# a-lemus96/fs-nerf

Hardware: AMD Instinct MI355X
Metric: rendered rays/sec (64+128 samples/ray, 8x256 MLP) (higher is better)
Workload: dtype fp16x3

## Files before the change

fs-nerf_amd/csrc/mlp_dev.hpp:

```cpp
#pragma once
#include "common.hpp"
#include "mlp_layout.hpp"
#ifndef FSN_KLOOP_HEADER
#define FSN_KLOOP_HEADER "kloop_gen.hpp"
#endif
#include FSN_KLOOP_HEADER

#include <type_traits>
#include <utility>

namespace fsn {

typedef __attribute__((ext_vector_type(8))) __bf16 bf16x8;
typedef __attribute__((ext_vector_type(8))) _Float16 f16x8;
typedef __attribute__((ext_vector_type(8))) short s16x8;
typedef __attribute__((ext_vector_type(4))) float f32x4;

constexpr int kNSlot = 4;
constexpr int kLead = 2;
constexpr int kLook = 2;
static_assert(kNSlot >= kLook + 2, "ring safety");
constexpr int kLoaders = 4;
constexpr int kLoaderXor = 4;
constexpr int kOpenVmcnt = (kLook - 1) * (kPhaseBytes / 1024 / kLoaders);
// ... 233 lines not shown
  }
}

constexpr uint32_t kSmallBits = 0x0400u;

struct RangeState {
  uint32_t fmax;
  uint32_t fall;
  uint32_t small;
};

constexpr uint32_t kSmallBitsU = 0x2c00u;

template <bool SMALL, uint32_t BITS = kSmallBits>
__device__ __forceinline__ void range_layer_end(RangeState& r) {
  asm("v_pk_max_u16 %0, %0, %1" : "+v"(r.fall) : "v"(r.fmax));
  if constexpr (SMALL) {
    const uint32_t lo = r.fmax & 0xffffu, hi = r.fmax >> 16;
    const uint32_t m = lo > hi ? lo : hi;
    const int any_big = __builtin_amdgcn_readfirstlane((int)__any(m >= BITS));
    const int any_nz = __builtin_amdgcn_readfirstlane((int)__any(m != 0u));
    if (!any_big && any_nz) r.small = 1u;
  }
  r.fmax = 0u;
}

__device__ __forceinline__ void range_report(uint32_t* status, const RangeState& r, uint32_t range_bit = 1u) {
  const uint32_t f = r.fall;
  const bool bad = (f & 0xffffu) >= 0x7c00u || (f >> 16) >= 0x7c00u;
  uint32_t bits = __builtin_amdgcn_readfirstlane((int)__any(bad)) ? range_bit : 0u;
  if (__builtin_amdgcn_readfirstlane((int)r.small)) bits |= 2u;
  if (bits && status) { if ((threadIdx.x & 63) == 0) __hip_atomic_fetch_or(status, bits, __ATOMIC_RELAXED, __HIP_MEMORY_SCOPE_AGENT); }
}

struct NetParams {
  const char* blob;
  int32_t aux_off, aux_floats, stream_off;
  int32_t nph_density, nph_full;
  int32_t n_layers;
  uint32_t skip_mask;
  int32_t n_freqs_pos, n_freqs_dir;
  uint32_t* status;
};

inline NetParams net_params(const fsn_mlp_desc& d, const NetGeom& G, const void* blob, uint32_t* status) {
  NetParams p;
  p.blob = static_cast<const char*>(blob);
  p.aux_off = (int32_t)G.aux_off; p.aux_floats = G.aux_floats; p.stream_off = (int32_t)G.stream_off;
  p.nph_density = G.nph_density; p.nph_full = G.nph_full;
  p.n_layers = d.n_layers; p.skip_mask = d.skip_mask;
  p.n_freqs_pos = d.n_freqs_pos; p.n_freqs_dir = d.n_freqs_dir;
  p.status = status;
  return p;
}

template <int... MODES>
struct PrecModes {};
template <int... MODES, class F>
inline int dispatch_net(PrecModes<MODES...>, int d_hidden, int prec, F&& f) {
  int rc = FSN_E_UNSUPPORTED;
  auto mode = [&](auto PREC) {
    if (prec != decltype(PREC)::value) return false;
    if (d_hidden == 256) rc = f(std::integral_constant<int, 8>{}, PREC);
    else if (d_hidden == 128) rc = f(std::integral_constant<int, 4>{}, PREC);
    return true;
  };
  (void)(mode(std::integral_constant<int, MODES>{}) || ...);
  return rc;
}
template <int... MODES, class F>
inline int dispatch_prec(PrecModes<MODES...>, int prec, F&& f) {
  int rc = FSN_E_UNSUPPORTED;
  auto mode = [&](auto PREC) { return prec == decltype(PREC)::value && (rc = f(PREC), true); };
  (void)(mode(std::integral_constant<int, MODES>{}) || ...);
  return rc;
}
using PrecInference = PrecModes<FSN_PREC_BF16X3, FSN_PREC_BF16, FSN_PREC_FP16X3, FSN_PREC_FP16, FSN_PREC_FP16X3U, FSN_PREC_FP16X2>;
using PrecTraining = PrecModes<FSN_PREC_BF16X3, FSN_PREC_BF16, FSN_PREC_FP16X3, FSN_PREC_FP16>;

struct NetDev {
  const float* aux;
  const float* pos_mask;
  const float* dir_mask;
  int32_t n_layers;
  uint32_t skip_mask;
  int32_t n_freqs_pos, n_freqs_dir;
  uint32_t* status;
};

__device__ __forceinline__ void sincos_f32(float a, float& s_out, float& c_out) {
  const float n = rintf(a * 0.63661977236758134f);
  float r = __builtin_fmaf(-n, 1.57079625129699707031e+00f, a);
  r = __builtin_fmaf(-n, 7.54978941586159635335e-08f, r);
  r = __builtin_fmaf(-n, 5.39030252995776476554e-15f, r);
  const float r2 = r * r;
  float ps = __builtin_fmaf(r2, -1.9515295891e-4f, 8.3321608736e-3f);
  ps = __builtin_fmaf(r2, ps, -1.6666654611e-1f);
  const float sn = __builtin_fmaf(r * r2, ps, r);
  float pc = __builtin_fmaf(r2, 2.443315711809948e-5f, -1.388731625493765e-3f);
  pc = __builtin_fmaf(r2, pc, 4.166664568298827e-2f);
  const float cs = __builtin_fmaf(r2 * r2, pc, __builtin_fmaf(r2, -0.5f, 1.0f));
  const int q = (int)n & 3;
  const float s1 = (q & 1) ? cs : sn;
  const float c1 = (q & 1) ? sn : cs;
  s_out = (q & 2) ? -s1 : s1;
  c_out = ((q + 1) & 2) ? -c1 : c1;
}

template <int NKS, bool F16, bool X3, bool SAVE = false, bool LS = (F16 && X3)>
__device__ __forceinline__ void encode(float x0, float x1, float x2, int n_freqs, const float* __restrict__ freqs,
                                       const float* __restrict__ mask, int g, Frag (&out)[NKS], uint32_t* save = nullptr) {
  constexpr int SLOTS = 8 * NKS;
  float v[SLOTS];
  const int P = 3 * n_freqs;
#pragma unroll
  for (int i = 0; i < SLOTS / 2; ++i) {
    const int p = 4 * i + g;
    const bool ok = p < P;
    const int ps = ok ? p : 0;
    const int band = (ps * 11) >> 5;
    const int coord = ps - 3 * band;
    const float xc = coord == 0 ? x0 : (coord == 1 ? x1 : x2);
    float s, c;
    if constexpr (X3) {
      sincos_f32(xc * freqs[band], s, c);
    } else {
      const float rev = (xc * freqs[band]) * 0.15915494309189535f;
      const float fr = __builtin_amdgcn_fractf(rev);
      s = __builtin_amdgcn_sinf(fr);
      c = __builtin_amdgcn_cosf(fr);
    }
    v[2 * i] = ok ? s * mask[3 + band * 6 + coord] : 0.f;
    v[2 * i + 1] = ok ? c * mask[3 + band * 6 + 3 + coord] : 0.f;
  }
  if (g == 2) {
    v[SLOTS - 2] = x0 * mask[0];
    v[SLOTS - 1] = x1 * mask[1];
  }
  if (g == 3) v[SLOTS - 2] = x2 * mask[2];
#pragma unroll
  for (int k = 0; k < NKS; ++k) split_store<F16, X3, LS>(&v[8 * k], out[k]);
  if constexpr (SAVE) {
    typedef __attribute__((ext_vector_type(4))) uint32_t u32x4;
    typedef __attribute__((ext_vector_type(2))) uint32_t u32x2;
#pragma unroll
    for (int k = 0; k < NKS; ++k) {
      const u32x4 h = __builtin_bit_cast(u32x4, out[k].hi), l = __builtin_bit_cast(u32x4, out[k].lo);
#pragma unroll
      for (int i = 0; i < 4; ++i) {
        if (X3) __builtin_nontemporal_store((u32x2){h[i], l[i]}, reinterpret_cast<u32x2*>(save + (16 * k + i) * kTRow * 2));
        else __builtin_nontemporal_store(h[i], save + (16 * k + i) * kTRow);
      }
    }
  }
}

enum : int { EPI_RELU_CVT = 0, EPI_LAST_FULL = 1, EPI_LAST_DENS = 4, EPI_CVT = 2, EPI_RGB = 3, EPI_NONE = 5 };

struct Heads {
  float sigma;
  float rgb[3];
  RangeState rs;
};

template <bool F16>
__device__ __forceinline__ f32x4 mfma16(const s16x8& a, const s16x8& b, const f32x4& c) {
  if (F16)
    return __builtin_amdgcn_mfma_f32_16x16x32_f16(__builtin_bit_cast(f16x8, a), __builtin_bit_cast(f16x8, b), c, 0, 0, 0);
  return __builtin_amdgcn_mfma_f32_16x16x32_bf16(__builtin_bit_cast(bf16x8, a), __builtin_bit_cast(bf16x8, b), c, 0, 0, 0);
}
struct AFrag {
  s16x8 hi, lo;
};
constexpr int kKD = FSN_KLOOP_D;
constexpr int kNS = FSN_KLOOP_NSETS;
struct ARing {
  AFrag cur[kNS > 3 ? kNS : 3];
};
template <int PREC>
__device__ __forceinline__ void load_afrag(const char* p, AFrag& f) {
  f.hi = *reinterpret_cast<const s16x8*>(p);
  if (prec_reads_w_lo(PREC)) f.lo = *reinterpret_cast<const s16x8*>(p + 1024);
}
template <int PREC>
__device__ __forceinline__ void unit_mfma_r(const AFrag& a, const Frag& b, f32x4& acc, f32x4& cor) {
  constexpr bool F16 = prec_is_f16(PREC), X3 = prec_is_x3(PREC);
  acc = mfma16<F16>(a.hi, b.hi, acc);
  if (X3) {
    f32x4& c = prec_one_acc(PREC) ? acc : cor;
    if (prec_reads_w_lo(PREC)) c = mfma16<F16>(a.lo, b.hi, c);
    c = mfma16<F16>(a.hi, b.lo, c);
  }
}

template <int PREC>
__device__ __forceinline__ void unit_mfma(const char* ubase, const Frag& b, f32x4& acc, f32x4& cor) {
  constexpr bool F16 = prec_is_f16(PREC), X3 = prec_is_x3(PREC);
  const s16x8 ah = *reinterpret_cast<const s16x8*>(ubase);
  acc = mfma16<F16>(ah, b.hi, acc);
  if (X3) {
    f32x4& c = prec_one_acc(PREC) ? acc : cor;
    if (prec_reads_w_lo(PREC)) {
      const s16x8 al = *reinterpret_cast<const s16x8*>(ubase + 1024);
      c = mfma16<F16>(al, b.hi, c);
    }
    c = mfma16<F16>(ah, b.lo, c);
  }
}

__device__ __forceinline__ float relu_f32(float v) {
  const int b = __builtin_bit_cast(int, v);
  return __builtin_bit_cast(float, b < 0 ? 0 : b);
}

struct NoHook {
  static constexpr bool kZeroInit = false;
  static constexpr bool kPacked = false;
  static constexpr bool kLayerEnd = false;
  __device__ __forceinline__ void pre(int) {}
  __device__ __forceinline__ void post(int, float (&)[8]) {}
};

// ... 355 lines not shown
    const f32x4 b0 = *reinterpret_cast<const f32x4*>(bias + 32 * tp + 4 * g);
    const f32x4 b1 = *reinterpret_cast<const f32x4*>(bias + 32 * tp + 16 + 4 * g);
    f32x4 a00 = b0, a01 = b1, a10 = b0, a11 = b1;
#pragma unroll
    for (int ks = 0; ks < KS; ++ks) {
      const Frag& x0 = ks < KS_ACT ? act[0][ks < KS_ACT ? ks : 0] : enc[0][ks >= KS_ACT ? ks - KS_ACT : 0];
      const Frag& x1 = ks < KS_ACT ? act[1][ks < KS_ACT ? ks : 0] : enc[1][ks >= KS_ACT ? ks - KS_ACT : 0];
      const int u = (tp * KS + ks) * 2;
      if (((u + kLead) % UPP == 0 && u + kLead <= TOTAL) || (u + kLead == TOTAL && TOTAL % UPP != 0)) st.open_next();
      if (u % UPP == 0) st.enter_phase();
      AFrag nxt[2];
      const int v = u + 2;
      const char* src = (v < TOTAL) ? ((v / UPP == u / UPP) ? st.c_base : st.n_base) + (v % UPP) * UB
                                    : st.n_base + (v - TOTAL) * UB;
      load_afrag<PREC>(src, nxt[0]);
      load_afrag<PREC>(src + UB, nxt[1]);
      a00 = mfma16<F16>(ring.cur[0].hi, x0.hi, a00);
      a10 = mfma16<F16>(ring.cur[0].hi, x1.hi, a10);
      a01 = mfma16<F16>(ring.cur[1].hi, x0.hi, a01);
      a11 = mfma16<F16>(ring.cur[1].hi, x1.hi, a11);
      ring.cur[0] = nxt[0];
      ring.cur[1] = nxt[1];
      __builtin_amdgcn_sched_group_barrier(0x100, 2, 0);
      __builtin_amdgcn_sched_group_barrier(0x008, 4, 0);
      __builtin_amdgcn_sched_barrier(0);
    }
    pair_epilogue<PREC, NP_OUT, EPI>(net, tp, a00, a01, a00, a01, out[0], heads[0], g, hk);
    pair_epilogue<PREC, NP_OUT, EPI>(net, tp, a10, a11, a10, a11, out[1], heads[1], g, hk);
  }
}

template <int PREC, int NT = 0>
__device__ __forceinline__ void prime_ring(const WStream& st, ARing& ring) {
  constexpr int UB = prec_is_x3(PREC) ? 2048 : 1024;
  if (kKloopAsm && prec_is_x3(PREC) && NT == 8) {
#pragma unroll
    for (int i = 0; i < kKD; ++i) load_afrag<PREC>(st.n_base + i * UB, ring.cur[i]);
#pragma unroll
    for (int i = kKD; i < (kNS > 3 ? kNS : 3); ++i) ring.cur[i] = ring.cur[0];
    return;
  }
#ifdef FSN_X3_PF1
  if (prec_is_x3(PREC)) {
    load_afrag<PREC>(st.n_base, ring.cur[0]);
    return;
  }
#else
  if (prec_is_x3(PREC)) return;
#endif
  load_afrag<PREC>(st.n_base, ring.cur[0]);
  load_afrag<PREC>(st.n_base + UB, ring.cur[1]);
  if (!prec_is_x3(PREC)) ring.cur[0].lo = ring.cur[1].lo = ring.cur[0].hi;
}

struct NoSave {
  static constexpr bool kSave = false;
  using Hook = NoHook;
  __device__ __forceinline__ Hook hidden(int) const { return {}; }
  __device__ __forceinline__ Hook branch() const { return {}; }
  __device__ __forceinline__ uint32_t* enc_pos(int) const { return nullptr; }
  __device__ __forceinline__ uint32_t* enc_dir(int) const { return nullptr; }
  __device__ __forceinline__ void layer_done(int, Hook&) const {}
};

#define FSN_PER_GROUP(Q, ...)               \
  do {                                      \
    {                                       \
      constexpr int Q = 0;                  \
      __VA_ARGS__                           \
    }                                       \
    if constexpr (NG == 2) {                \
      constexpr int Q = NG - 1;             \
      __VA_ARGS__                           \
    }                                       \
  } while (0)

#define FSN_TEMPLATE_ARGS(...) __VA_ARGS__
#define FSN_GEMM_LAYER(TA, BIAS, IN, ENC, OUT)                                                                          \
  do {                                                                                                                  \
    if constexpr (NG == 1) gemm_layer<FSN_TEMPLATE_ARGS TA>(st, net, BIAS, IN[0], ENC[0], OUT[0], heads[0], ring, g, hk); \
    else gemm_layer_two_groups<FSN_TEMPLATE_ARGS TA>(st, net, BIAS, IN, ENC, OUT, heads, ring, g);                       \
  } while (0)

template <int NT, int PREC, bool FULL, int NG, class Src, class SV>
__device__ __forceinline__ void mlp_tile(WStream& st, const NetDev& net, const Src (&src)[NG], ARing& ring,
                                         float (&sigma)[NG], float (&rgb)[NG][3], const SV& sv) {
  constexpr int NA = NT;
  constexpr bool F16 = prec_is_f16(PREC), X3 = prec_is_x3(PREC), LS = prec_lo_scaled(PREC);
  static_assert(NG == 1 || (NG == 2 && !X3 && std::is_same<SV, NoSave>::value), "sample groups per wave");
  const int g = (threadIdx.x >> 4) & 3;
  constexpr int D = 32 * NT;
  const int L = net.n_layers;
  const float* misc = net.aux + (L + 5) * D;
  Frag A[NG][NA], B[NG][NA];
  Frag none[NG][1];
  Heads heads[NG];
  FSN_PER_GROUP(q, heads[q] = Heads{0.f, {0.f, 0.f, 0.f}, {0u, 0u, 0u}};);
#define FSN_ENC_POS(SAVE, PE)                                                                                 \
  FSN_PER_GROUP(q, float px, py, pz; src[q].pos(px, py, pz);                                                     \
                encode<kKsPos, F16, X3, SAVE, LS>(px, py, pz, net.n_freqs_pos, misc + 4, net.pos_mask, g, PE[q], \
                                                  SAVE ? sv.enc_pos(g) : nullptr);)
  {
    Frag pe[NG][kKsPos];
    FSN_ENC_POS(SV::kSave, pe);
    typename SV::Hook hk = sv.hidden(0);
    FSN_GEMM_LAYER((PREC, NT, 0, kKsPos, EPI_RELU_CVT), 0, none, pe, A);
    sv.layer_done(0, hk);
  }
#define FSN_HIDDEN(EPI, IN, OUT, LIDX)                                                              \
  do {                                                                                              \
    typename SV::Hook hk = sv.hidden(LIDX);                                                         \
    if ((net.skip_mask >> ((LIDX)-1)) & 1u) {                                                       \
      Frag pe2[NG][kKsPos];                                                                         \
      FSN_ENC_POS(false, pe2);                                                                      \
      FSN_GEMM_LAYER((PREC, NT, NA, kKsPos, EPI), (LIDX)*D, IN, pe2, OUT);   \
    } else                                                                                          \
      FSN_GEMM_LAYER((PREC, NT, NA, 0, EPI), (LIDX)*D, IN, none, OUT);       \
    sv.layer_done(LIDX, hk);                                                                        \
  } while (0)
  for (int l = 1; l <= L - 2; l += 2) {
    FSN_HIDDEN(EPI_RELU_CVT, A, B, l);
    if (l + 1 <= L - 2) {
      FSN_HIDDEN(EPI_RELU_CVT, B, A, l + 1);
    } else {
      FSN_PER_GROUP(q, Frag(&a)[NA] = A[q]; const Frag(&b)[NA] = B[q];
                    _Pragma("unroll") for (int i = 0; i < NA; ++i) a[i] = b[i];);
    }
  }
  FSN_HIDDEN((FULL ? EPI_LAST_FULL : EPI_LAST_DENS), A, B, L - 1);
#undef FSN_HIDDEN
#undef FSN_ENC_POS
  {
    float sg[NG];
    FSN_PER_GROUP(q, sg[q] = heads[q].sigma;);
    FSN_PER_GROUP(q, sg[q] += __shfl_xor(sg[q], 16, 64););
    FSN_PER_GROUP(q, sg[q] += __shfl_xor(sg[q], 32, 64););
    FSN_PER_GROUP(q, sigma[q] = sg[q] + misc[0];);
  }
  if (FULL) {
    {
      typename SV::Hook hk = sv.hidden(L);
      FSN_GEMM_LAYER((PREC, NT, NA, 0, EPI_CVT), L * D, B, none, A);
      sv.layer_done(L, hk);
    }
    Frag de[NG][kKsDir];
    FSN_PER_GROUP(q, float dx, dy, dz; src[q].dir(dx, dy, dz);
                  encode<kKsDir, F16, X3, SV::kSave, LS>(dx, dy, dz, net.n_freqs_dir, misc + 20, net.dir_mask, g, de[q], sv.enc_dir(g)););
    {
      typename SV::Hook hk = sv.branch();
      FSN_GEMM_LAYER((PREC, NT / 2, NA, kKsDir, EPI_RGB), (L + 1) * D, A, de, B);
      sv.layer_done(L + 1, hk);
    }
#pragma unroll
    for (int c = 0; c < 3; ++c) {
      float z[NG];
      FSN_PER_GROUP(q, z[q] = heads[q].rgb[c];);
      FSN_PER_GROUP(q, z[q] += __shfl_xor(z[q], 16, 64););
      FSN_PER_GROUP(q, z[q] += __shfl_xor(z[q], 32, 64););
      FSN_PER_GROUP(q, z[q] += misc[1 + c]; rgb[q][c] = 1.0f / (1.0f + expf(-z[q])););
    }
  }
  if constexpr (F16) {
    if constexpr (NG == 2) asm("v_pk_max_u16 %0, %0, %1" : "+v"(heads[0].rs.fmax) : "v"(heads[1].rs.fmax));
    range_layer_end<false>(heads[0].rs);
    range_report(net.status, heads[0].rs);
  }
}

#undef FSN_GEMM_LAYER
#undef FSN_TEMPLATE_ARGS

template <int NT, int PREC, bool FULL, int NG, class Src>
__device__ __forceinline__ void mlp_tile(WStream& st, const NetDev& net, const Src (&src)[NG], ARing& ring,
                                         float (&sigma)[NG], float (&rgb)[NG][3]) {
  mlp_tile<NT, PREC, FULL>(st, net, src, ring, sigma, rgb, NoSave{});
}

struct TileSrc {
  const float* p;
  __device__ __forceinline__ void pos(float& x, float& y, float& z) const { x = p[0]; y = p[1]; z = p[2]; }
  __device__ __forceinline__ void dir(float& x, float& y, float& z) const { x = p[3]; y = p[4]; z = p[5]; }
};

__device__ __forceinline__ void ray_sample(const float* __restrict__ ro, const float* __restrict__ rd,
                                           const int64_t* __restrict__ ri, const float* __restrict__ t0,
                                           const float* __restrict__ t1, int64_t s, float* q, bool with_dir) {
  const int64_t r = ri[s];
  const float tm = t0[s] + t1[s];
#pragma unroll
  for (int c = 0; c < 3; ++c) {
    const float dc = rd[3 * r + c];
    q[c] = ro[3 * r + c] + dc * tm / 2.0f;
    if (with_dir) q[3 + c] = dc;
  }
}

__device__ __forceinline__ void load_net(const NetParams& p, const float* __restrict__ pos_mask_g,
                                         const float* __restrict__ dir_mask_g, float* lds, NetDev& net) {
  const f32x4* src = reinterpret_cast<const f32x4*>(p.blob + p.aux_off);
  f32x4* dst = reinterpret_cast<f32x4*>(lds);
  for (int i = threadIdx.x; i < p.aux_floats / 4; i += blockDim.x) dst[i] = src[i];
  float* pm = lds + p.aux_floats;
  float* dm = pm + 64;
  const int npe = 3 * (1 + 2 * p.n_freqs_pos), nde = 3 * (1 + 2 * p.n_freqs_dir);
  for (int i = threadIdx.x; i < 64; i += blockDim.x) pm[i] = (pos_mask_g && i < npe) ? pos_mask_g[i] : 1.0f;
  for (int i = threadIdx.x; i < 32; i += blockDim.x) dm[i] = (dir_mask_g && i < nde) ? dir_mask_g[i] : 1.0f;
  net.aux = lds;
  net.pos_mask = pm;
  net.dir_mask = dm;
  net.n_layers = p.n_layers;
  net.skip_mask = p.skip_mask;
  net.n_freqs_pos = p.n_freqs_pos;
  net.n_freqs_dir = p.n_freqs_dir;
  net.status = p.status;
}

}
```

fs-nerf_amd/csrc/render.hip:

```cpp
#include "common.hpp"
#define FSN_KLOOP_ASM
#define FSN_BF16X3_ONEACC 1
#include "mlp_dev.hpp"
#include "ray_dev.hpp"

namespace fsn {

FSN_DEBUG_DEFINE_RECORD(g_dbg_render)
#define FSN_DEBUG_RECORD g_dbg_render

constexpr int kMaxGroupSamples = 768;
constexpr int kMaxGroupCoarse = 768;
constexpr int kMaxG = 4;
constexpr int kMaxRaySamples = 384;
struct RenderKArgs {
  NetParams netC, netF;
  fsn_render_args a;
  int32_t G, nsubC, nsubF;
  float step;
  int32_t two_phase;
  float cam_hw, cam_hh, cam_f;
};

struct RenderLds {
  fsn_render_args args;
  int32_t Gc, nsubC, nsubF;
  float step;
  int32_t two_phase;
  float cam_hw, cam_hh, cam_f;
  float rays[kMaxG * 6];
  float edgesC[kMaxGroupCoarse + kMaxG];
  float sigC[kMaxGroupCoarse];
  float wC[kMaxGroupCoarse];
  float edgesF[kMaxGroupSamples + kMaxG];
  float sigF[kMaxGroupSamples];
  float rgbF[3 * kMaxGroupSamples];
  float cdf[kMaxG][kMaxRaySamples + 1];
  float vals[kMaxG][kMaxRaySamples + 1];
};

constexpr int kNetLdsBytes = (kAuxCapFloats + 96) * 4;
constexpr int kRenderLdsBytes = kRingBytes + 2 * kNetLdsBytes + (int)sizeof(RenderLds);
static_assert(kRenderLdsBytes <= 160 * 1024, "LDS budget");

struct RaySrc {
  const float* ray;
  const float* e;
  __device__ __forceinline__ void pos(float& x, float& y, float& z) const {
    const float tm = e[0] + e[1];
    x = ray[0] + ray[3] * tm / 2.0f;
    y = ray[1] + ray[4] * tm / 2.0f;
    z = ray[2] + ray[5] * tm / 2.0f;
  }
  __device__ __forceinline__ void dir(float& x, float& y, float& z) const { x = ray[3]; y = ray[4]; z = ray[5]; }
};

#define GRP_S (a.S)
#define GRP_NI (a.n_imp)
#define GRP_SO (a.S + a.n_imp)
#define GRP_HIER (a.n_imp > 0)
#define GRP_G (S_.Gc)
#define GRP_R (a.R)
#ifdef FSN_STAMP
__device__ unsigned long long g_stamp[256 * 8 * 8];
#endif
template <int NT, int PREC, bool TWO_PHASE>
__global__ __launch_bounds__(kThreads) void k_render_fused(RenderKArgs k) {
#ifdef FSN_STAMP
  const uint64_t t_begin = __builtin_amdgcn_s_memtime();
#endif
  uint64_t clk_t0 = 0, clk_r0 = 0;
  const bool clk_on = k.a.clock_out != nullptr && blockIdx.x == 0 && __builtin_amdgcn_readfirstlane(threadIdx.x) < 64;
  if (clk_on) { clk_t0 = __builtin_amdgcn_s_memtime(); clk_r0 = __builtin_amdgcn_s_memrealtime(); }
  auto clk_end = [&]() __attribute__((always_inline)) {
    if (clk_on && (threadIdx.x & 63) == 0) {
      k.a.clock_out[0] += __builtin_amdgcn_s_memtime() - clk_t0;
      k.a.clock_out[1] += __builtin_amdgcn_s_memrealtime() - clk_r0;
    }
  };
  __shared__ __attribute__((aligned(1024))) char smem[kRenderLdsBytes];
  float* auxC = reinterpret_cast<float*>(smem + kRingBytes);
  float* auxF = reinterpret_cast<float*>(smem + kRingBytes + kNetLdsBytes);
  RenderLds& S_ = *reinterpret_cast<RenderLds*>(smem + kRingBytes + 2 * kNetLdsBytes);
  if (threadIdx.x == 0) S_.args = k.a;
  __syncthreads();
  const fsn_render_args& a = S_.args;
  if (threadIdx.x == 0) {
    S_.Gc = k.G; S_.nsubC = k.nsubC; S_.nsubF = k.nsubF; S_.step = k.step; S_.two_phase = k.two_phase;
    S_.cam_hw = k.cam_hw; S_.cam_hh = k.cam_hh; S_.cam_f = k.cam_f;
  }
  __syncthreads();
  NetDev netC, netF;
  load_net(k.netF, a.pos_mask, a.dir_mask, auxF, netF);
  if (GRP_HIER) load_net(k.netC, a.pos_mask, a.dir_mask, auxC, netC);
  else netC = netF;
  __syncthreads();
  WStream st;
  {
    const int64_t ngr = (k.a.R + k.G - 1) / k.G;
    const int64_t mine = ngr > (int64_t)blockIdx.x ? (ngr - blockIdx.x + gridDim.x - 1) / gridDim.x : 0;
    const uint32_t repC = k.two_phase ? (uint32_t)(mine * k.nsubC) : (uint32_t)k.nsubC;
    const uint32_t repF = k.two_phase == 2 ? 0u : (k.two_phase ? (uint32_t)(mine * k.nsubF) : (uint32_t)k.nsubF);
    st.init(smem, k.netC.blob + k.netC.stream_off, GRP_HIER ? (uint32_t)k.netC.nph_density : 0u, repC,
            k.netF.blob + k.netF.stream_off, (uint32_t)k.netF.nph_full, repF);
  }
  int tid = threadIdx.x, wave = tid >> 6, lane = tid & 63;
#define FSN_RELAUNDER()                                              \
  do {                                                               \
    int t_ = threadIdx.x;                                            \
    asm volatile("" : "+v"(t_));                                     \
    tid = t_; wave = __builtin_amdgcn_readfirstlane(t_ >> 6); lane = t_ & 63; \
  } while (0)
  constexpr int NG = groups_per_wave<NT, PREC>(), TILE = 128 * NG;
  ARing ring;
  prime_ring<PREC, NT>(st, ring);
  auto small_div = [](int n, int d) __attribute__((always_inline)) {
    int q = (int)(((float)n + 0.5f) * __builtin_amdgcn_rcpf((float)d));
    q += (q + 1) * d <= n ? 1 : 0;
    q -= q * d > n ? 1 : 0;
    return q;
  };
  auto load_rays = [&](int64_t r0) __attribute__((always_inline)) {
    if (a.rays_o) {
      if (tid < GRP_G * 6) {
        const int g = tid / 6, c = tid - 6 * g;
        const int64_t ray = min(r0 + g, GRP_R - 1);
        FSN_AT(S_.rays, tid) = c < 3 ? a.rays_o[3 * ray + c] : a.rays_d[3 * ray + c - 3];
      }
    } else if (tid < GRP_G) {
      const int64_t ray = min(r0 + tid, GRP_R - 1);
      const uint32_t Wc = (uint32_t)__builtin_amdgcn_readfirstlane(a.cam_W), rr = (uint32_t)ray;
      const int h = a.cam_row0 + (int)(rr / Wc), w = (int)(rr % Wc);
      float o[3], d[3];
      pinhole_ray(a.cam_pose, S_.cam_hw, S_.cam_hh, S_.cam_f, h, w, o, d);
#pragma unroll
      for (int c = 0; c < 3; ++c) { FSN_AT(S_.rays, 6 * tid + c) = o[c]; FSN_AT(S_.rays, 6 * tid + 3 + c) = d[c]; }
    }
  };
  auto coarse_stage = [&](int64_t r0) __attribute__((always_inline)) {
    for (int e = tid; e < GRP_G * (GRP_S + 1); e += kThreads) {
      const int g = small_div(e, GRP_S + 1), i = e - g * (GRP_S + 1);
      const int64_t ray = min(r0 + g, GRP_R - 1);
      const float* ur = a.u_mode == 1 ? a.u + ray : (a.u_mode == 2 ? a.u + ray * (GRP_S + 1) : nullptr);
      FSN_AT(S_.edgesC, e) = stratified_edge(a.near, S_.step, GRP_S, i, a.u_mode, ur);
    }
    lds_barrier();
    if (!GRP_HIER) return;
    st.pass_begin();
    for (int sub = 0; sub < S_.nsubC; ++sub) {
      auto slot = [&](int q) { return sub * TILE + tile_slot<NG>(wave, lane, q); };
      auto source = [&](int idx) {
        const int idc = min(idx, GRP_G * GRP_S - 1);
        const int g = small_div(idc, GRP_S), i = idc - g * GRP_S;
        return RaySrc{FSN_SPAN(S_.rays, 6 * g, 6), FSN_SPAN(S_.edgesC, g * (GRP_S + 1) + i, 2)};
      };
      const int idx0 = slot(0);
      RaySrc src[NG];
      FSN_PER_GROUP(q, src[q] = source(idx0 + 16 * q););
      float sigma[NG], rgb[NG][3];
      mlp_tile<NT, PREC, false>(st, netC, src, ring, sigma, rgb);
      if (tile_stores<NG>(lane)) {
        const int qs = tile_store_group<NG>(lane), idx = idx0 + 16 * qs;
        if (idx < GRP_G * GRP_S) FSN_AT(S_.sigC, idx) = sigma[qs];
      }
    }
    st.pass_end();
    lds_barrier();
    for (int g = wave; g < GRP_G; g += kWaves) {
      const int64_t ray = min(r0 + g, GRP_R - 1);
      float* wc = FSN_SPAN(S_.wC, g * GRP_S, GRP_S);
      weights_ray(FSN_SPAN(S_.sigC, g * GRP_S, GRP_S), FSN_SPAN(S_.edgesC, g * (GRP_S + 1), GRP_S + 1), GRP_S, wc);
      __builtin_amdgcn_wave_barrier();
      if (a.weights_coarse && r0 + g < GRP_R)
        for (int i = lane; i < GRP_S; i += 64) a.weights_coarse[ray * GRP_S + i] = wc[i];
      sample_pdf_merge_ray(FSN_SPAN(S_.edgesC, g * (GRP_S + 1), GRP_S + 1), wc, GRP_S, GRP_NI,
                           a.u_fine ? a.u_fine + ray * GRP_NI : nullptr, FSN_AT(S_.cdf, g), FSN_AT(S_.vals, g),
                           FSN_SPAN(S_.edgesF, g * (GRP_SO + 1), GRP_SO + 1));
    }
    lds_barrier();
  };
  auto fine_stage = [&](int64_t r0, const float* edges, bool write_edges) __attribute__((always_inline)) {
    st.pass_begin();
    for (int sub = 0; sub < S_.nsubF; ++sub) {
      auto slot = [&](int q) { return sub * TILE + tile_slot<NG>(wave, lane, q); };
      auto source = [&](int idx) {
        const int idc = min(idx, GRP_G * GRP_SO - 1);
        const int g = small_div(idc, GRP_SO), i = idc - g * GRP_SO;
        return RaySrc{FSN_SPAN(S_.rays, 6 * g, 6), edges + g * (GRP_SO + 1) + i};
      };
      const int idx0 = slot(0);
      RaySrc src[NG];
      FSN_PER_GROUP(q, src[q] = source(idx0 + 16 * q););
      float sigma[NG], rgb[NG][3];
      mlp_tile<NT, PREC, true>(st, netF, src, ring, sigma, rgb);
      if (tile_stores<NG>(lane)) {
        const int qs = tile_store_group<NG>(lane), idx = idx0 + 16 * qs;
        if (idx < GRP_G * GRP_SO) {
          FSN_AT(S_.sigF, idx) = sigma[qs];
          FSN_AT(S_.rgbF, 3 * idx + 0) = rgb[qs][0];
          FSN_AT(S_.rgbF, 3 * idx + 1) = rgb[qs][1];
          FSN_AT(S_.rgbF, 3 * idx + 2) = rgb[qs][2];
        }
      }
    }
    st.pass_end();
    lds_barrier();
    for (int g = wave; g < GRP_G; g += kWaves) {
      if (r0 + g >= GRP_R) continue;
      const int64_t ray = r0 + g;
      const float* eg = edges + g * (GRP_SO + 1);
      CompositeOut o{a.colors + 3 * ray, a.opacity + ray, a.depth + ray,
                     a.weights ? a.weights + ray * GRP_SO : nullptr, a.alphas ? a.alphas + ray * GRP_SO : nullptr,
                     a.trans ? a.trans + ray * GRP_SO : nullptr};
      composite_ray(FSN_SPAN(S_.sigF, g * GRP_SO, GRP_SO), FSN_SPAN(S_.rgbF, 3 * g * GRP_SO, 3 * GRP_SO), eg, eg + 1, GRP_SO,
                    true, a.bkgd[0], a.bkgd[1], a.bkgd[2], o);
      if (a.sigmas)
        for (int i = lane; i < GRP_SO; i += 64) a.sigmas[ray * GRP_SO + i] = FSN_AT(S_.sigF, g * GRP_SO + i);
      if (a.rgbs)
        for (int i = lane; i < 3 * GRP_SO; i += 64) a.rgbs[ray * GRP_SO * 3 + i] = FSN_AT(S_.rgbF, 3 * g * GRP_SO + i);
      if (write_edges && a.edges_out)
        for (int i = lane; i <= GRP_SO; i += 64) a.edges_out[ray * (GRP_SO + 1) + i] = eg[i];
    }
    lds_barrier();
  };
  const int64_t ngroups = (GRP_R + GRP_G - 1) / GRP_G;
  if constexpr (!TWO_PHASE) {
    for (int64_t grp = blockIdx.x; grp < ngroups; grp += gridDim.x) {
      FSN_RELAUNDER();
      const int64_t r0 = grp * (int64_t)__builtin_amdgcn_readfirstlane(GRP_G);
      load_rays(r0);
      coarse_stage(r0);
      fine_stage(r0, GRP_HIER ? FSN_SPAN(S_.edgesF, 0, GRP_G * (GRP_SO + 1)) : FSN_SPAN(S_.edgesC, 0, GRP_G * (GRP_SO + 1)), true);
    }
  } else {
    for (int64_t grp = blockIdx.x; grp < ngroups; grp += gridDim.x) {
      FSN_RELAUNDER();
      const int64_t r0 = grp * (int64_t)__builtin_amdgcn_readfirstlane(GRP_G);
      load_rays(r0);
      coarse_stage(r0);
      for (int e = tid; e < GRP_G * (GRP_SO + 1); e += kThreads) {
        const int g = small_div(e, GRP_SO + 1), i = e - g * (GRP_SO + 1);
        if (r0 + g < GRP_R) __builtin_nontemporal_store(FSN_AT(S_.edgesF, e), a.edges_out + (r0 + g) * (GRP_SO + 1) + i);
      }
      lds_barrier();
    }
    __builtin_amdgcn_fence(__ATOMIC_RELEASE, "workgroup");
    __syncthreads();
    __builtin_amdgcn_fence(__ATOMIC_ACQUIRE, "workgroup");
    if (S_.two_phase == 2) {
      st.drain();
      clk_end();
      return;
    }
    for (int64_t grp = blockIdx.x; grp < ngroups; grp += gridDim.x) {
      FSN_RELAUNDER();
      const int64_t r0 = grp * (int64_t)__builtin_amdgcn_readfirstlane(GRP_G);
      load_rays(r0);
      for (int e = tid; e < GRP_G * (GRP_SO + 1); e += kThreads) {
        const int g = small_div(e, GRP_SO + 1), i = e - g * (GRP_SO + 1);
        FSN_AT(S_.edgesF, e) = __builtin_nontemporal_load(a.edges_out + min(r0 + g, GRP_R - 1) * (GRP_SO + 1) + i);
      }
      lds_barrier();
      fine_stage(r0, FSN_SPAN(S_.edgesF, 0, GRP_G * (GRP_SO + 1)), false);
    }
  }
  st.drain();
  clk_end();
#ifdef FSN_STAMP
  if ((threadIdx.x & 63) == 0 && blockIdx.x < 256) {
    unsigned long long* o = g_stamp + (blockIdx.x * 8 + (threadIdx.x >> 6)) * 8;
    o[0] = __builtin_amdgcn_s_memtime() - t_begin; o[1] = st.t_k; o[2] = st.t_e; o[3] = st.t_n;
    o[4] = st.t_ko; o[5] = st.t_eo;
  }
#endif
}

template <int PREC>
__global__ __launch_bounds__(kThreads) void k_bare_stream(const char* stream, uint32_t nph, int layers, uint64_t* clk) {
  __shared__ __attribute__((aligned(1024))) char smem[kRingBytes + 256 * 4];
  float* zeros = reinterpret_cast<float*>(smem + kRingBytes);
  for (int i = threadIdx.x; i < 256; i += blockDim.x) zeros[i] = 0.f;
  __syncthreads();
  NetDev net{};
  net.aux = zeros;
  net.n_layers = 8;
  WStream st;
  st.init(smem, nullptr, 0, 0, stream, nph, 1);
  ARing ring;
  prime_ring<PREC, 8>(st, ring);
  const int g = (threadIdx.x >> 4) & 3;
  Frag A[8], B[8];
  Frag none[1];
  uint32_t h = 0x9e3779b9u * (threadIdx.x + 1u) + 0x85ebca6bu * (blockIdx.x + 1u);
  auto next = [&]() { h ^= h << 13; h ^= h >> 17; h ^= h << 5; return h; };
#pragma unroll
  for (int k = 0; k < 8; ++k)
#pragma unroll
    for (int j = 0; j < 8; ++j) {
      const uint32_t r = next();
      const uint16_t hi = (r & 1u) ? (uint16_t)(0x3c00u + ((r >> 1) % 9u) * 0x0400u + ((r >> 8) & 0x3ffu)) : (uint16_t)0;
      const uint16_t lo = (r & 1u) ? (uint16_t)((hi - 0x2c00u) ^ ((r >> 20) & 0x8000u)) : (uint16_t)0;
      A[k].hi[j] = (short)hi;
      A[k].lo[j] = (short)lo;
    }
  Heads heads{0.f, {0.f, 0.f, 0.f}, {0u, 0u, 0u}};
  const uint64_t t0 = __builtin_amdgcn_s_memtime(), r0 = __builtin_amdgcn_s_memrealtime();
  for (int l = 0; l < layers; ++l) {
    gemm_layer<PREC, 8, 8, 0, EPI_RELU_CVT>(st, net, 0, A, none, B, heads, ring, g);
    asm volatile("" ::"v"(B[0].hi), "v"(B[7].lo));
  }
  const uint64_t t1 = __builtin_amdgcn_s_memtime(), r1 = __builtin_amdgcn_s_memrealtime();
  st.drain();
  if (clk && (threadIdx.x & 63) == 0) {
    uint64_t* o = clk + 2 * (blockIdx.x * kWaves + (threadIdx.x >> 6));
    o[0] = t1 - t0;
    o[1] = r1 - r0;
  }
  if (heads.rs.fall == 0xffffffffu && clk) clk[0] = 0;
}

#undef GRP_S
#undef GRP_NI
#undef GRP_SO
#undef GRP_HIER
#undef GRP_G
#undef GRP_R

template <int NT, int PREC>
static int launch_render(RenderKArgs k, int cus, hipStream_t s) {
  constexpr int kTilesG1 = 2;
  constexpr int NG = groups_per_wave<NT, PREC>(), TILE = 128 * NG, CAP = NG == 1 ? 384 * kTilesG1 : kMaxGroupSamples;
  const int So = k.a.S + k.a.n_imp;
  int g = (NG == 1 ? kTilesG1 : 1) * TILE / k.a.S;
  if (g < 1) g = 1;
  if (g > CAP / So) g = CAP / So;
  if (g > kMaxG) g = kMaxG;
  if (g > kMaxGroupCoarse / k.a.S) g = kMaxGroupCoarse / k.a.S;
  if (g < 1) g = 1;
  k.G = g;
  k.nsubC = (g * k.a.S + TILE - 1) / TILE;
// ... 136 lines not shown
```

Before: 1.598 million.

## Cache direction encodings per ray, stash positional encoding in LDS, skip unit masks

```diff
diff --git a/fs-nerf_amd/csrc/mlp_dev.hpp b/fs-nerf_amd/csrc/mlp_dev.hpp
--- a/fs-nerf_amd/csrc/mlp_dev.hpp
+++ b/fs-nerf_amd/csrc/mlp_dev.hpp
@@ -339,6 +339,7 @@
   const float* aux;
   const float* pos_mask;
   const float* dir_mask;
+  bool pos_masked;
   int32_t n_layers;
   uint32_t skip_mask;
   int32_t n_freqs_pos, n_freqs_dir;
@@ -364,7 +365,7 @@
   c_out = ((q + 1) & 2) ? -c1 : c1;
 }
 
-template <int NKS, bool F16, bool X3, bool SAVE = false, bool LS = (F16 && X3)>
+template <int NKS, bool F16, bool X3, bool SAVE = false, bool LS = (F16 && X3), bool MASKED = true>
 __device__ __forceinline__ void encode(float x0, float x1, float x2, int n_freqs, const float* __restrict__ freqs,
                                        const float* __restrict__ mask, int g, Frag (&out)[NKS], uint32_t* save = nullptr) {
   constexpr int SLOTS = 8 * NKS;
@@ -387,14 +388,19 @@
       s = __builtin_amdgcn_sinf(fr);
       c = __builtin_amdgcn_cosf(fr);
     }
-    v[2 * i] = ok ? s * mask[3 + band * 6 + coord] : 0.f;
-    v[2 * i + 1] = ok ? c * mask[3 + band * 6 + 3 + coord] : 0.f;
+    if constexpr (MASKED) {
+      v[2 * i] = ok ? s * mask[3 + band * 6 + coord] : 0.f;
+      v[2 * i + 1] = ok ? c * mask[3 + band * 6 + 3 + coord] : 0.f;
+    } else {
+      v[2 * i] = ok ? s : 0.f;
+      v[2 * i + 1] = ok ? c : 0.f;
+    }
   }
   if (g == 2) {
-    v[SLOTS - 2] = x0 * mask[0];
-    v[SLOTS - 1] = x1 * mask[1];
-  }
-  if (g == 3) v[SLOTS - 2] = x2 * mask[2];
+    v[SLOTS - 2] = MASKED ? x0 * mask[0] : x0;
+    v[SLOTS - 1] = MASKED ? x1 * mask[1] : x1;
+  }
+  if (g == 3) v[SLOTS - 2] = MASKED ? x2 * mask[2] : x2;
 #pragma unroll
   for (int k = 0; k < NKS; ++k) split_store<F16, X3, LS>(&v[8 * k], out[k]);
   if constexpr (SAVE) {
@@ -916,11 +922,34 @@
     else gemm_layer_two_groups<FSN_TEMPLATE_ARGS TA>(st, net, BIAS, IN, ENC, OUT, heads, ring, g);                       \
   } while (0)
 
+template <class S, class = void>
+struct src_skips_unit_mask : std::false_type {};
+template <class S>
+struct src_skips_unit_mask<S, std::enable_if_t<S::kSkipUnitMask>> : std::true_type {};
+template <class S, class = void>
+struct src_has_dir_frag : std::false_type {};
+template <class S>
+struct src_has_dir_frag<S, std::void_t<decltype(&S::dir_frag)>> : std::true_type {};
+template <class S, class = void>
+struct src_has_pos_stash : std::false_type {};
+template <class S>
+struct src_has_pos_stash<S, std::void_t<decltype(&S::stash_pos), decltype(&S::fetch_pos)>> : std::true_type {};
+
+template <int NT, int PREC>
+__device__ __forceinline__ void encode_dir(const NetDev& net, float dx, float dy, float dz, int g, Frag (&de)[kKsDir]) {
+  const float* misc = net.aux + (net.n_layers + 5) * (32 * NT);
+  encode<kKsDir, prec_is_f16(PREC), prec_is_x3(PREC), false, prec_lo_scaled(PREC)>(dx, dy, dz, net.n_freqs_dir, misc + 20,
+                                                                                   net.dir_mask, g, de);
+}
+
 template <int NT, int PREC, bool FULL, int NG, class Src, class SV>
 __device__ __forceinline__ void mlp_tile(WStream& st, const NetDev& net, const Src (&src)[NG], ARing& ring,
                                          float (&sigma)[NG], float (&rgb)[NG][3], const SV& sv) {
   constexpr int NA = NT;
   constexpr bool F16 = prec_is_f16(PREC), X3 = prec_is_x3(PREC), LS = prec_lo_scaled(PREC);
+  constexpr bool kDirFrag = X3 && src_has_dir_frag<Src>::value, kPosStash = X3 && src_has_pos_stash<Src>::value;
+  constexpr bool kUnitMask = X3 && NG == 1 && !SV::kSave && src_skips_unit_mask<Src>::value;
+  static_assert(!(kDirFrag || kPosStash) || (NG == 1 && !SV::kSave), "encoding reuse: one group, nothing saved");
   static_assert(NG == 1 || (NG == 2 && !X3 && std::is_same<SV, NoSave>::value), "sample groups per wave");
   const int g = (threadIdx.x >> 4) & 3;
   constexpr int D = 32 * NT;
@@ -936,7 +965,20 @@
                                                   SAVE ? sv.enc_pos(g) : nullptr);)
   {
     Frag pe[NG][kKsPos];
-    FSN_ENC_POS(SV::kSave, pe);
+    if constexpr (kUnitMask) {
+      if (net.pos_masked) {
+        FSN_ENC_POS(false, pe);
+      } else {
+        float px, py, pz;
+        src[0].pos(px, py, pz);
+        encode<kKsPos, F16, X3, false, LS, false>(px, py, pz, net.n_freqs_pos, misc + 4, net.pos_mask, g, pe[0]);
+      }
+    } else {
+      FSN_ENC_POS(SV::kSave, pe);
+    }
+    if constexpr (kPosStash) {
+      if (net.skip_mask) src[0].stash_pos(pe[0]);
+    }
     typename SV::Hook hk = sv.hidden(0);
     FSN_GEMM_LAYER((PREC, NT, 0, kKsPos, EPI_RELU_CVT), 0, none, pe, A);
     sv.layer_done(0, hk);
@@ -946,7 +988,11 @@
     typename SV::Hook hk = sv.hidden(LIDX);                                                         \
     if ((net.skip_mask >> ((LIDX)-1)) & 1u) {                                                       \
       Frag pe2[NG][kKsPos];                                                                         \
-      FSN_ENC_POS(false, pe2);                                                                      \
+      if constexpr (kPosStash) {                                                                    \
+        src[0].fetch_pos(pe2[0]);                                                                   \
+      } else {                                                                                      \
+        FSN_ENC_POS(false, pe2);                                                                    \
+      }                                                                                             \
       FSN_GEMM_LAYER((PREC, NT, NA, kKsPos, EPI), (LIDX)*D, IN, pe2, OUT);   \
     } else                                                                                          \
       FSN_GEMM_LAYER((PREC, NT, NA, 0, EPI), (LIDX)*D, IN, none, OUT);       \
@@ -978,8 +1024,12 @@
       sv.layer_done(L, hk);
     }
     Frag de[NG][kKsDir];
-    FSN_PER_GROUP(q, float dx, dy, dz; src[q].dir(dx, dy, dz);
-                  encode<kKsDir, F16, X3, SV::kSave, LS>(dx, dy, dz, net.n_freqs_dir, misc + 20, net.dir_mask, g, de[q], sv.enc_dir(g)););
+    if constexpr (kDirFrag) {
+      src[0].dir_frag(de[0][0]);
+    } else {
+      FSN_PER_GROUP(q, float dx, dy, dz; src[q].dir(dx, dy, dz);
+                    encode<kKsDir, F16, X3, SV::kSave, LS>(dx, dy, dz, net.n_freqs_dir, misc + 20, net.dir_mask, g, de[q], sv.enc_dir(g)););
+    }
     {
       typename SV::Hook hk = sv.branch();
       FSN_GEMM_LAYER((PREC, NT / 2, NA, kKsDir, EPI_RGB), (L + 1) * D, A, de, B);
@@ -1042,6 +1092,7 @@
   net.aux = lds;
   net.pos_mask = pm;
   net.dir_mask = dm;
+  net.pos_masked = __builtin_amdgcn_readfirstlane(pos_mask_g != nullptr) != 0;
   net.n_layers = p.n_layers;
   net.skip_mask = p.skip_mask;
   net.n_freqs_pos = p.n_freqs_pos;
diff --git a/fs-nerf_amd/csrc/render.hip b/fs-nerf_amd/csrc/render.hip
--- a/fs-nerf_amd/csrc/render.hip
+++ b/fs-nerf_amd/csrc/render.hip
@@ -29,23 +29,71 @@
   int32_t two_phase;
   float cam_hw, cam_hh, cam_f;
   float rays[kMaxG * 6];
+  alignas(16) Frag dirF[kMaxG][4];
   float edgesC[kMaxGroupCoarse + kMaxG];
   float sigC[kMaxGroupCoarse];
-  float wC[kMaxGroupCoarse];
   float edgesF[kMaxGroupSamples + kMaxG];
   float sigF[kMaxGroupSamples];
   float rgbF[3 * kMaxGroupSamples];
-  float cdf[kMaxG][kMaxRaySamples + 1];
-  float vals[kMaxG][kMaxRaySamples + 1];
+  union {
+    struct {
+      float wC[kMaxGroupCoarse];
+      float cdf[kMaxG][kMaxRaySamples + 1];
+      float vals[kMaxG][kMaxRaySamples + 1];
+    };
+    s16x8 stash[2 * kKsPos][kThreads];
+  };
 };
 
 constexpr int kNetLdsBytes = (kAuxCapFloats + 96) * 4;
 constexpr int kRenderLdsBytes = kRingBytes + 2 * kNetLdsBytes + (int)sizeof(RenderLds);
 static_assert(kRenderLdsBytes <= 160 * 1024, "LDS budget");
+static_assert((kRingBytes + 2 * kNetLdsBytes) % 16 == 0 && alignof(RenderLds) == 16, "dirF / stash: 16-byte LDS accesses");
+
+#ifndef FSN_ENC_DIR_TABLE
+#define FSN_ENC_DIR_TABLE 1
+#endif
+#ifndef FSN_ENC_POS_STASH
+#define FSN_ENC_POS_STASH 1
+#endif
+#ifndef FSN_ENC_UNIT_MASK_SKIP
+#define FSN_ENC_UNIT_MASK_SKIP 1
+#endif
 
 struct RaySrc {
   const float* ray;
   const float* e;
+  const Frag* dfr;
+  RenderLds* lds;
+#if FSN_ENC_UNIT_MASK_SKIP
+  static constexpr bool kSkipUnitMask = true;
+#endif
+#if FSN_ENC_DIR_TABLE
+  __device__ __forceinline__ void dir_frag(Frag& f) const { f = *dfr; }
+#endif
+#if FSN_ENC_POS_STASH
+  static __device__ __forceinline__ int stash_column() {
+    int t = threadIdx.x;
+    asm volatile("" : "+v"(t));
+    return t;
+  }
+  __device__ __forceinline__ void stash_pos(const Frag (&pe)[kKsPos]) const {
+    const int t = stash_column();
+#pragma unroll
+    for (int k = 0; k < kKsPos; ++k) {
+      FSN_AT(FSN_AT(lds->stash, 2 * k), t) = pe[k].hi;
+      FSN_AT(FSN_AT(lds->stash, 2 * k + 1), t) = pe[k].lo;
+    }
+  }
+  __device__ __forceinline__ void fetch_pos(Frag (&pe)[kKsPos]) const {
+    const int t = stash_column();
+#pragma unroll
+    for (int k = 0; k < kKsPos; ++k) {
+      pe[k].hi = FSN_AT(FSN_AT(lds->stash, 2 * k), t);
+      pe[k].lo = FSN_AT(FSN_AT(lds->stash, 2 * k + 1), t);
+    }
+  }
+#endif
   __device__ __forceinline__ void pos(float& x, float& y, float& z) const {
     const float tm = e[0] + e[1];
     x = ray[0] + ray[3] * tm / 2.0f;
@@ -137,6 +185,18 @@
       for (int c = 0; c < 3; ++c) { FSN_AT(S_.rays, 6 * tid + c) = o[c]; FSN_AT(S_.rays, 6 * tid + 3 + c) = d[c]; }
     }
   };
+  auto fill_dir_frags = [&]() __attribute__((always_inline)) {
+    if constexpr (FSN_ENC_DIR_TABLE && prec_is_x3(PREC)) {
+      lds_barrier();
+      if (tid < 4 * GRP_G) {
+        const int r = tid >> 2;
+        const float* ray = FSN_SPAN(S_.rays, 6 * r, 6);
+        Frag de[kKsDir];
+        encode_dir<NT, PREC>(netF, ray[3], ray[4], ray[5], tid & 3, de);
+        FSN_AT(FSN_AT(S_.dirF, r), tid & 3) = de[0];
+      }
+    }
+  };
   auto coarse_stage = [&](int64_t r0) __attribute__((always_inline)) {
     for (int e = tid; e < GRP_G * (GRP_S + 1); e += kThreads) {
       const int g = small_div(e, GRP_S + 1), i = e - g * (GRP_S + 1);
@@ -152,7 +212,7 @@
       auto source = [&](int idx) {
         const int idc = min(idx, GRP_G * GRP_S - 1);
         const int g = small_div(idc, GRP_S), i = idc - g * GRP_S;
-        return RaySrc{FSN_SPAN(S_.rays, 6 * g, 6), FSN_SPAN(S_.edgesC, g * (GRP_S + 1) + i, 2)};
+        return RaySrc{FSN_SPAN(S_.rays, 6 * g, 6), FSN_SPAN(S_.edgesC, g * (GRP_S + 1) + i, 2), nullptr, &S_};
       };
       const int idx0 = slot(0);
       RaySrc src[NG];
@@ -186,7 +246,7 @@
       auto source = [&](int idx) {
         const int idc = min(idx, GRP_G * GRP_SO - 1);
         const int g = small_div(idc, GRP_SO), i = idc - g * GRP_SO;
-        return RaySrc{FSN_SPAN(S_.rays, 6 * g, 6), edges + g * (GRP_SO + 1) + i};
+        return RaySrc{FSN_SPAN(S_.rays, 6 * g, 6), edges + g * (GRP_SO + 1) + i, &FSN_AT(FSN_AT(S_.dirF, g), lane >> 4), &S_};
       };
       const int idx0 = slot(0);
       RaySrc src[NG];
@@ -229,6 +289,7 @@
       FSN_RELAUNDER();
       const int64_t r0 = grp * (int64_t)__builtin_amdgcn_readfirstlane(GRP_G);
       load_rays(r0);
+      fill_dir_frags();
       coarse_stage(r0);
       fine_stage(r0, GRP_HIER ? FSN_SPAN(S_.edgesF, 0, GRP_G * (GRP_SO + 1)) : FSN_SPAN(S_.edgesC, 0, GRP_G * (GRP_SO + 1)), true);
     }
@@ -256,6 +317,7 @@
       FSN_RELAUNDER();
       const int64_t r0 = grp * (int64_t)__builtin_amdgcn_readfirstlane(GRP_G);
       load_rays(r0);
+      fill_dir_frags();
       for (int e = tid; e < GRP_G * (GRP_SO + 1); e += kThreads) {
         const int g = small_div(e, GRP_SO + 1), i = e - g * (GRP_SO + 1);
         FSN_AT(S_.edgesF, e) = __builtin_nontemporal_load(a.edges_out + min(r0 + g, GRP_R - 1) * (GRP_SO + 1) + i);
```

New measurement: 1.634 million, median of 6. +2.3%, better.
